# Peyton-Chen/RegionE

Hardware: AMD Instinct MI355X
Metric: denoising steps/sec (28-step RegionE edit, 1024x1024) (higher is better)
Workload: dtype bf16

## Files before the change

### regione_amd/_lib.py

```python
from __future__ import annotations

import ctypes as C
import os

import torch

from . import build as _build
from .build import LIB_PATH

LIB_PATH = os.environ.get("RGN_LIB", LIB_PATH)

_c_void_p, _c_int, _c_float = C.c_void_p, C.c_int, C.c_float



class QkvEpilogue(C.Structure):
    _fields_ = [("wq", _c_void_p), ("wk", _c_void_p), ("cos_q", _c_void_p), ("sin_q", _c_void_p), ("cos_k", _c_void_p),
                ("sin_k", _c_void_p), ("kv_rows", _c_void_p), ("k_slab", _c_void_p), ("vt_slab", _c_void_p),
                ("row_base", _c_int), ("skv_pad", _c_int), ("k_col", _c_int), ("v_col", _c_int), ("q_col", _c_int),
                ("heads", _c_int), ("eps", _c_float), ("fp16_roundtrip", _c_int)]


_qkv_p = C.POINTER(QkvEpilogue)

# ... 135 lines not shown
    "rgn_mmdit_double_block": [_block_p, _c_void_p],
    "rgn_mmdit_single_block": [_block_p, _c_void_p],
    "rgn_mmdit_block_bytes": [],
    "rgn_lora_merge_bf16": [_c_void_p, _c_int, _c_void_p, _c_int, _c_int, _c_int, _term_p, _c_int, _c_void_p],
    "rgn_image_resample_u8": [_c_void_p, _c_int, _c_int, _c_void_p, _c_int, _c_int, _c_void_p, _c_void_p, _c_int, _c_int, _c_void_p],
    "rgn_image_u8_to_nchw_bf16": [_c_void_p, _c_void_p, _c_int, _c_int, _c_void_p, _c_void_p],
    "rgn_image_patchify_u8": [_c_void_p, _c_int, _c_int, _c_void_p, _c_void_p, _c_int, _c_int, _c_void_p],
    "rgn_image_bf16_to_u8": [_c_void_p, _c_int, _c_int, _c_void_p, _c_int, _c_int, _c_void_p],
}
_RESTYPE = {"rgn_last_error": C.c_char_p, "rgn_abi_struct_bytes": C.c_size_t, "rgn_attention_workspace_bytes": C.c_size_t,
            "rgn_gemm_workspace_bytes": C.c_size_t, "rgn_groupnorm_workspace_bytes": C.c_size_t,
            "rgn_groupnorm_partial_bytes": C.c_size_t, "rgn_lm_decode_attention_workspace_bytes": C.c_size_t,
            "rgn_lm_head_workspace_bytes": C.c_size_t, "rgn_lm_pick_workspace_bytes": C.c_size_t,
            "rgn_rowband_side_launches": C.c_longlong, "rgn_mmdit_block_bytes": C.c_size_t}

_lib = None


class RegionEHipError(RuntimeError):
    pass


def lib():
    global _lib
    if _lib is not None:
        return _lib
    if not os.path.exists(LIB_PATH):
        raise RegionEHipError(
            f"{LIB_PATH} not found: the HIP extension is not built. Run "
            "`python -c 'import __graft_entry__ as g; g.build()'` (needs hipcc); there is no CPU fallback.")
    if os.path.abspath(LIB_PATH) == os.path.abspath(_build.LIB_PATH) and os.path.isdir(_build.CSRC):
        built, now = _build.built_from(), _build.csrc_hash()
        if built and built != now:
            raise RegionEHipError(f"{LIB_PATH} was built from kernel sources {built}, the tree holds {now}: rebuild with "
                                  "`python -m regione_amd.build` (or `__graft_entry__.build()`)")
    h = C.CDLL(LIB_PATH)
    for name, argtypes in SIGNATURES.items():
        fn = getattr(h, name)
        fn.argtypes = argtypes
        fn.restype = _RESTYPE.get(name, C.c_int)
    want = C.sizeof(QkvEpilogue) * 1000 + C.sizeof(GemmProblem)
    if h.rgn_abi_struct_bytes() != want:
        raise RegionEHipError(f"{LIB_PATH}: struct layout {h.rgn_abi_struct_bytes()} != the Python binding's {want} "
                              f"(library ABI version {h.rgn_version()}): rebuild with `python -m regione_amd.build --force`")
    if h.rgn_mmdit_block_bytes() != C.sizeof(MmditBlock):
        raise RegionEHipError(f"{LIB_PATH}: sizeof(rgn_mmdit_block) {h.rgn_mmdit_block_bytes()} != the Python binding's {C.sizeof(MmditBlock)}: "
                              "rebuild with `python -m regione_amd.build --force`")
    _lib = h
    return h


import contextlib as _contextlib

PLAN_KEYS = ("gemm_pieces", "gemm_geometry", "gemm_asm", "gemm_quarter", "attn_waves", "attn_split", "attn_streamk", "attn_asm", "rowbands")


@_contextlib.contextmanager
def plan_override(**knobs):
    h = lib()
    before = {}
    try:
        for k, v in knobs.items():
            old = C.c_int(-1)
            check(h.rgn_plan_override_get(k.encode(), C.byref(old)), f"rgn_plan_override_get({k})")
            check(h.rgn_plan_override(k.encode(), int(v)), f"rgn_plan_override({k})")
            before[k] = old.value
        yield
    finally:
        for k, old in before.items():
            h.rgn_plan_override(k.encode(), old)


def check(rc: int, what: str = ""):
    if rc != 0:
        msg = lib().rgn_last_error().decode(errors="replace")
        raise RegionEHipError(f"{what or 'libregione_hip'} failed (rc={rc}): {msg}")
```

### regione_amd/csrc/attn.hip

```cpp
#include "common.h"
#include <stdlib.h>
#include <utility>
#include "attn_loop_asm.inc"

namespace rgn {

typedef __attribute__((ext_vector_type(8))) __bf16 bf8_t;
typedef __attribute__((ext_vector_type(2))) __bf16 bf2_t;
typedef __attribute__((ext_vector_type(2))) float f32x2;
typedef __attribute__((address_space(3))) void* lds_ptr_t;
typedef const __attribute__((address_space(1))) void* glb_ptr_t;

struct AttnArgs {
    const uint16_t* Q;
    const uint16_t* K;
    const uint16_t* Vt;
    uint16_t* O;
    int ldq, ldo, skv_pad, Sq, Skv, H;
    float scale_log2e;
    int item_offset, nitems_launch, nsplit;
    int static_on;
    float static_m;
    float* ws;
};
// ... 368 lines not shown
                         : RGN_ATTN_LOOP_CLOBBERS);
        }
    }
    const float l_other = __shfl_xor(l_run, 32, 64);
    const float l_tot = l_run + l_other;
    if (SPLIT) {
        const size_t slot = SPLIT == 2 ? (size_t)unit * 2 + seg : (size_t)(item - g.item_offset) * g.nsplit + split;
        float* base = g.ws + slot * (size_t)(QB * 130);
        float* orow = base + (size_t)(wave * 32 + ql) * 128;
        static_for<16>([&](auto Ic) {
            constexpr int I = decltype(Ic)::value;
            constexpr int db = I / 4, r4 = I % 4;
            *(float4*)(orow + db * 32 + 8 * r4 + 4 * half) =
                make_float4(agpr_read1<db * 16 + r4 * 4 + 0>(), agpr_read1<db * 16 + r4 * 4 + 1>(),
                            agpr_read1<db * 16 + r4 * 4 + 2>(), agpr_read1<db * 16 + r4 * 4 + 3>());
        });
        if (half == 0) {
            base[QB * 128 + wave * 32 + ql] = m_run;
            base[QB * 129 + wave * 32 + ql] = l_tot;
        }
        if (SPLIT != 2) return;
        sk_lo += ntiles;
        ++seg;
        if (sk_lo >= sk_hi) return;
        __syncthreads();
        continue;
    }
    const float inv = 1.0f / l_tot;
    constexpr int OT_LD = 136;
    uint16_t* ot = (uint16_t*)smem;
    {
        uint16_t* orow = ot + (wave * 32 + ql) * OT_LD;
        static_for<16>([&](auto Ic) {
            constexpr int I = decltype(Ic)::value;
            constexpr int db = I / 4, r4 = I % 4;
            const int d = db * 32 + 8 * r4 + 4 * half;
            const uint32_t w0 = cvt_pk_bf16(agpr_read1<db * 16 + r4 * 4 + 0>() * inv, agpr_read1<db * 16 + r4 * 4 + 1>() * inv);
            const uint32_t w1 = cvt_pk_bf16(agpr_read1<db * 16 + r4 * 4 + 2>() * inv, agpr_read1<db * 16 + r4 * 4 + 3>() * inv);
            *(uint2*)(orow + d) = make_uint2(w0, w1);
        });
    }
    __syncthreads();
    constexpr int RPP = 512 / 16;
#pragma unroll
    for (int it = 0; it < QB / RPP; ++it) {
        const int row = (tid >> 4) + it * RPP, c = (tid & 15) * 8;
        const int qr2 = qb * QB + row;
        if (qr2 < g.Sq) *(uint4*)(g.O + (size_t)qr2 * g.ldo + h * 128 + c) = *(const uint4*)(ot + row * OT_LD + c);
    }
    return;
  }
}

__global__ __launch_bounds__(256, 1) void attention_asm64_kernel(const AttnArgs g) {
    constexpr int QB = 256;
    extern __shared__ __attribute__((aligned(16))) uint8_t smem[];
    const int tid = threadIdx.x;
    const int wave = __builtin_amdgcn_readfirstlane(tid >> 6);
    const int nQ = (g.Sq + QB - 1) / QB;
    const int ntiles = g.Skv / KV_T;
    int unit;
    {
        const int nb = g.nitems_launch;
        const int bid = blockIdx.x, xcd = bid & 7, loc = bid >> 3;
        const int q = nb >> 3, r = nb & 7;
        unit = (xcd < r ? xcd * (q + 1) : r * (q + 1) + (xcd - r) * q) + loc;
    }
    const uint32_t HD2 = (uint32_t)g.H * 256u;
    const int lane = tid & 63;
    const int ql = lane & 31, half = lane >> 5;
    const int item = g.item_offset + unit;
    const int h = item / nQ, qb = item - h * nQ;
    const int q0 = qb * QB + wave * 64;
    float m_run = g.static_m, l_run0 = 0.f, l_run1 = 0.f;
    {
        uint32_t krel[8], vrel[4];
#pragma unroll
        for (int ks = 0; ks < 8; ++ks) krel[ks] = ql * 256 + (((ks * 2 + half) ^ (ql & 15)) << 4);
#pragma unroll
        for (int kb4 = 0; kb4 < 4; ++kb4) vrel[kb4] = ql * 128 + (((kb4 * 2 + half) ^ ((ql >> 1) & 7)) << 4);
        uint32_t dk[4], dv[4];
#pragma unroll
        for (int p = 0; p < 4; ++p) {
            const int piece = wave * 4 + p;
            const int krow = piece * 4 + (lane >> 4);
            dk[p] = (uint32_t)krow * HD2 + h * 256 + (((lane & 15) ^ (krow & 15)) << 4);
            const int vrow = piece * 8 + (lane >> 3);
            dv[p] = (uint32_t)(h * 128 + vrow) * (uint32_t)(g.skv_pad * 2) + (((lane & 7) ^ ((vrow >> 1) & 7)) << 4);
        }
        const uint16_t* qptr0 = g.Q + (size_t)min(q0 + ql, g.Sq - 1) * g.ldq + h * 128 + half * 8;
        const uint16_t* qptr1 = g.Q + (size_t)min(q0 + 32 + ql, g.Sq - 1) * g.ldq + h * 128 + half * 8;
        auto rsrc = [](const void* p) {
            const uint64_t a = (uint64_t)p;
            u32x4_s r;
            r[0] = __builtin_amdgcn_readfirstlane((uint32_t)a);
            r[1] = __builtin_amdgcn_readfirstlane((uint32_t)(a >> 32) & 0xffffu);
            r[2] = 0xffffffffu;
            r[3] = 0x00020000u;
            return r;
        };
        const u32x4_s rk = rsrc(g.K), rv = rsrc(g.Vt);
        const uint32_t lds0 = (uint32_t)(uintptr_t)(__attribute__((address_space(3))) uint8_t*)smem;
        const uint32_t kadv = __builtin_amdgcn_readfirstlane((uint32_t)KV_T * HD2);
        uint32_t tk = __builtin_amdgcn_readfirstlane(0u), tv = __builtin_amdgcn_readfirstlane(0u);
        const uint32_t tk_last = __builtin_amdgcn_readfirstlane((uint32_t)(ntiles - 1) * kadv);
        const uint32_t tv_last = __builtin_amdgcn_readfirstlane((uint32_t)(ntiles - 1) * 128u);
        uint32_t stg_k = __builtin_amdgcn_readfirstlane(lds0 + 32768u), stg_v = __builtin_amdgcn_readfirstlane(lds0), stg_d = stg_v;
        const uint32_t wdst = __builtin_amdgcn_readfirstlane((uint32_t)wave * 4096u);
        uint32_t cnt = __builtin_amdgcn_readfirstlane((uint32_t)(ntiles - 1) >> 1), rem = __builtin_amdgcn_readfirstlane((uint32_t)(ntiles - 1) & 1u);
        const float sl2e = g.scale_log2e;
        uint32_t stmp, stmp2, sdst;
        asm volatile(RGN_ATTN_LOOP_W64_ASM
                     : [l_run0] "+&v"(l_run0), [l_run1] "+&v"(l_run1), [tk] "+&s"(tk), [tv] "+&s"(tv), [stg_k] "+&s"(stg_k),
                       [stg_v] "+&s"(stg_v), [stg_d] "+&s"(stg_d), [cnt] "+&s"(cnt), [stmp] "=&s"(stmp), [stmp2] "=&s"(stmp2),
                       [sdst] "=&s"(sdst)
                     : [krel0] "v"(krel[0]), [krel1] "v"(krel[1]), [krel2] "v"(krel[2]), [krel3] "v"(krel[3]), [krel4] "v"(krel[4]),
                       [krel5] "v"(krel[5]), [krel6] "v"(krel[6]), [krel7] "v"(krel[7]), [vrel0] "v"(vrel[0]), [vrel1] "v"(vrel[1]),
                       [vrel2] "v"(vrel[2]), [vrel3] "v"(vrel[3]), [dk0] "v"(dk[0]), [dk1] "v"(dk[1]), [dk2] "v"(dk[2]), [dk3] "v"(dk[3]),
                       [dv0] "v"(dv[0]), [dv1] "v"(dv[1]), [dv2] "v"(dv[2]), [dv3] "v"(dv[3]), [qptr0] "v"(qptr0), [qptr1] "v"(qptr1),
                       [m_run] "v"(m_run), [rk] "s"(rk), [rv] "s"(rv), [kadv] "s"(kadv), [tk_last] "s"(tk_last), [tv_last] "s"(tv_last),
                       [wdst] "s"(wdst), [rem] "s"(rem), [sl2e] "s"(sl2e)
                     : RGN_ATTN_LOOP_W64_CLOBBERS);
    }
    const float inv0 = 1.0f / (l_run0 + __shfl_xor(l_run0, 32, 64));
    const float inv1 = 1.0f / (l_run1 + __shfl_xor(l_run1, 32, 64));
    constexpr int OT_LD = 136;
    uint16_t* ot = (uint16_t*)smem;
    static_for<32>([&](auto Ic) {
        constexpr int I = decltype(Ic)::value;
        constexpr int j = I / 16, db = (I / 4) % 4, r4 = I % 4, A = j * 64 + db * 16 + r4 * 4;
        const float inv = j ? inv1 : inv0;
        uint16_t* orow = ot + ((wave * 2 + j) * 32 + ql) * OT_LD;
        const int d = db * 32 + 8 * r4 + 4 * half;
        const uint32_t w0 = cvt_pk_bf16(agpr_read1<A + 0>() * inv, agpr_read1<A + 1>() * inv);
        const uint32_t w1 = cvt_pk_bf16(agpr_read1<A + 2>() * inv, agpr_read1<A + 3>() * inv);
        *(uint2*)(orow + d) = make_uint2(w0, w1);
    });
    __syncthreads();
    constexpr int RPP = 256 / 16;
#pragma unroll
    for (int it = 0; it < QB / RPP; ++it) {
        const int row = (tid >> 4) + it * RPP, c = (tid & 15) * 8;
        const int qr2 = qb * QB + row;
        if (qr2 < g.Sq) *(uint4*)(g.O + (size_t)qr2 * g.ldo + h * 128 + c) = *(const uint4*)(ot + row * OT_LD + c);
    }
}

template <int QB>
__global__ __launch_bounds__(256) void attention_combine_kernel(const AttnArgs g) {
    const int nQ = (g.Sq + QB - 1) / QB;
    const int u = blockIdx.x / (QB / 16);
    const int row = (blockIdx.x % (QB / 16)) * 16 + (threadIdx.x >> 4);
    const int c = (threadIdx.x & 15) * 8;
    const int item = g.item_offset + u;
    const int h = item / nQ, qb = item - h * nQ;
    const int qr = qb * QB + row;
    if (qr >= g.Sq) return;
    const float* base = g.ws + (size_t)u * g.nsplit * (size_t)(QB * 130);
    float mstar = -1e30f;
    for (int s = 0; s < g.nsplit; ++s) mstar = fmaxf(mstar, base[(size_t)s * QB * 130 + QB * 128 + row]);
    float acc[8] = {0.f, 0.f, 0.f, 0.f, 0.f, 0.f, 0.f, 0.f};
    float l = 0.f;
    for (int s = 0; s < g.nsplit; ++s) {
        const float* b = base + (size_t)s * QB * 130;
        const float w = __builtin_amdgcn_exp2f(b[QB * 128 + row] - mstar);
        l += b[QB * 129 + row] * w;
        const float4 x0 = *(const float4*)(b + (size_t)row * 128 + c), x1 = *(const float4*)(b + (size_t)row * 128 + c + 4);
        acc[0] += x0.x * w; acc[1] += x0.y * w; acc[2] += x0.z * w; acc[3] += x0.w * w;
        acc[4] += x1.x * w; acc[5] += x1.y * w; acc[6] += x1.z * w; acc[7] += x1.w * w;
    }
    const float inv = 1.0f / l;
    uint4 out;
    out.x = cvt_pk_bf16(acc[0] * inv, acc[1] * inv); out.y = cvt_pk_bf16(acc[2] * inv, acc[3] * inv);
    out.z = cvt_pk_bf16(acc[4] * inv, acc[5] * inv); out.w = cvt_pk_bf16(acc[6] * inv, acc[7] * inv);
    *(uint4*)(g.O + (size_t)qr * g.ldo + h * 128 + c) = out;
}

template <int QB>
__global__ __launch_bounds__(256) void attention_combine_sk_kernel(const AttnArgs g, int G) {
    const int nQ = (g.Sq + QB - 1) / QB;
    const int u = blockIdx.x / (QB / 16);
    const int row = (blockIdx.x % (QB / 16)) * 16 + (threadIdx.x >> 4);
    const int c = (threadIdx.x & 15) * 8;
    const int item = g.item_offset + u;
    const int h = item / nQ, qb = item - h * nQ;
    const int qr = qb * QB + row;
    if (qr >= g.Sq) return;
    const int nt = g.Skv / KV_T;
    const long long total = (long long)g.nitems_launch * nt;
    const long long lo = (long long)u * nt, hi = lo + nt;
    auto bound = [&](int w) { return (long long)w * total / G; };
    int w0 = (int)(lo * G / total);
    while (w0 + 1 < G && bound(w0 + 1) <= lo) ++w0;
    while (w0 > 0 && bound(w0) > lo) --w0;
    float mstar = -1e30f;
    for (int w = w0; w < G && bound(w) < hi; ++w) {
        if (bound(w + 1) <= bound(w)) continue;
        const int sg = ((int)(bound(w) / nt) == u) ? 0 : 1;
        mstar = fmaxf(mstar, g.ws[((size_t)w * 2 + sg) * (size_t)(QB * 130) + QB * 128 + row]);
    }
    float acc[8] = {0.f, 0.f, 0.f, 0.f, 0.f, 0.f, 0.f, 0.f};
    float l = 0.f;
    for (int w = w0; w < G && bound(w) < hi; ++w) {
        if (bound(w + 1) <= bound(w)) continue;
        const int sg = ((int)(bound(w) / nt) == u) ? 0 : 1;
        const float* b = g.ws + ((size_t)w * 2 + sg) * (size_t)(QB * 130);
        const float wt = __builtin_amdgcn_exp2f(b[QB * 128 + row] - mstar);
        l += b[QB * 129 + row] * wt;
        const float4 x0 = *(const float4*)(b + (size_t)row * 128 + c), x1 = *(const float4*)(b + (size_t)row * 128 + c + 4);
        acc[0] += x0.x * wt; acc[1] += x0.y * wt; acc[2] += x0.z * wt; acc[3] += x0.w * wt;
        acc[4] += x1.x * wt; acc[5] += x1.y * wt; acc[6] += x1.z * wt; acc[7] += x1.w * wt;
    }
    const float inv = 1.0f / l;
    uint4 out;
    out.x = cvt_pk_bf16(acc[0] * inv, acc[1] * inv); out.y = cvt_pk_bf16(acc[2] * inv, acc[3] * inv);
    out.z = cvt_pk_bf16(acc[4] * inv, acc[5] * inv); out.w = cvt_pk_bf16(acc[6] * inv, acc[7] * inv);
    *(uint4*)(g.O + (size_t)qr * g.ldo + h * 128 + c) = out;
}

template <int SPLIT>
static int launch_attention_asm(const AttnArgs& g, int nblocks, hipStream_t st) {
    constexpr int LDS = 5 * ATT_STAGE;
    static bool attr[64] = {};
    int dev = 0;
    (void)hipGetDevice(&dev);
    if (dev < 0 || dev >= 64 || !attr[dev]) {
        (void)hipFuncSetAttribute((const void*)attention_asm_kernel<SPLIT, false>, hipFuncAttributeMaxDynamicSharedMemorySize, LDS);
        (void)hipFuncSetAttribute((const void*)attention_asm_kernel<SPLIT, true>, hipFuncAttributeMaxDynamicSharedMemorySize, LDS);
        if (SPLIT == 0) (void)hipFuncSetAttribute((const void*)attention_asm64_kernel, hipFuncAttributeMaxDynamicSharedMemorySize, LDS);
        if (dev >= 0 && dev < 64) attr[dev] = true;
    }
    if (nblocks == 0) return 0;
    if (SPLIT == 0 && g.static_on) hipLaunchKernelGGL(attention_asm64_kernel, dim3(nblocks), dim3(256), LDS, st, g);
    else if (g.static_on) hipLaunchKernelGGL((attention_asm_kernel<SPLIT, true>), dim3(nblocks), dim3(512), LDS, st, g);
    else hipLaunchKernelGGL((attention_asm_kernel<SPLIT, false>), dim3(nblocks), dim3(512), LDS, st, g);
    return check_launch("attention_asm_kernel");
}

static bool attention_use_asm(const AttnArgs& g) {
    return plan_override().attn_asm != 0 && (g.Skv % KV_T) == 0 && (size_t)g.skv_pad * g.H * 256 < ((size_t)1 << 32);
}

template <int NW, int NSTAGE, bool SPLIT>
static int launch_attention(const AttnArgs& g, hipStream_t st) {
    if (NW == 8 && attention_use_asm(g))
        return launch_attention_asm<SPLIT ? 1 : 0>(g, SPLIT ? g.nitems_launch * g.nsplit : g.nitems_launch, st);
    constexpr int LDS = NSTAGE * ATT_STAGE;
    static bool attr[64] = {};
    int dev = 0;
    (void)hipGetDevice(&dev);
    if (dev < 0 || dev >= 64 || !attr[dev]) {
        (void)hipFuncSetAttribute((const void*)attention_kernel<NW, NSTAGE, SPLIT>, hipFuncAttributeMaxDynamicSharedMemorySize, LDS);
        if (dev >= 0 && dev < 64) attr[dev] = true;
    }
    const int nblocks = SPLIT ? g.nitems_launch * g.nsplit : g.nitems_launch;
    if (nblocks == 0) return 0;
    hipLaunchKernelGGL((attention_kernel<NW, NSTAGE, SPLIT>), dim3(nblocks), dim3(64 * NW), LDS, st, g);
    return check_launch("attention_kernel");
}

static thread_local int g_last_attn_plan = 0;

template <int NW, int NSTAGE>
static int attention_schedule(AttnArgs g, int slots, void* ws, size_t ws_bytes, hipStream_t st, bool dry = false) {
    constexpr int QB = 32 * NW;
    const int nitems = g.H * ((g.Sq + QB - 1) / QB);
    const int ntiles = (g.Skv + KV_T - 1) / KV_T;
    int full = (nitems / slots) * slots, left = nitems - full, best = 1;
    const float c_t = NW == 8 ? 1.69f : 0.95f, c_p = 10.7f, c_m = 8.0f;
    float best_cost = (float)((left + slots - 1) / slots) * ((float)ntiles * c_t + c_p);
    if (NW == 8 && full == 0 && left > 0) {
        const float x = fmaxf(0.0f, (float)(left - 72) / 184.0f);
        best_cost = (float)ntiles * (1.10f + 0.59f * x * x) + c_p;
    }
    bool stream_k = false;
    if (left > 0 && ws != nullptr) {
        for (int S = 2; S <= 8; ++S) {
            if (ntiles / S < 4) break;
            if ((size_t)left * S * QB * 130 * sizeof(float) > ws_bytes) break;
            const float cost = (float)((left * S + slots - 1) / slots) * ((float)((ntiles + S - 1) / S) * c_t + c_p) + c_m;
            if (cost < best_cost - 1e-3f) { best_cost = cost; best = S; }
        }
        const int sk_o = plan_override().attn_streamk;
        const long long steps = (long long)left * ntiles;
        if (NW == 8 && sk_o != 0 && attention_use_asm(g) && left < slots && steps >= 8LL * slots &&
            (size_t)slots * 2 * QB * 130 * sizeof(float) <= ws_bytes) {
            const float cost = (float)((steps + slots - 1) / slots) * c_t + 2.0f * c_p + c_m;
            if (cost < best_cost - 1e-3f || sk_o == 1) { best_cost = cost; stream_k = true; }
        }
    }
    g_last_attn_plan = (stream_k ? 1 : best) | (stream_k ? 0x10 : 0) | (NW == 8 ? 0x20 : 0);
    if (dry) return 0;
    g.ws = (float*)ws;
    g.nsplit = 1;
    int rc = 0;
    if (stream_k) {
        if (full > 0) {
            g.item_offset = 0; g.nitems_launch = full;
            if ((rc = launch_attention<NW, NSTAGE, false>(g, st))) return rc;
        }
        g.item_offset = full; g.nitems_launch = left;
        if ((rc = launch_attention_asm<2>(g, slots, st))) return rc;
        hipLaunchKernelGGL((attention_combine_sk_kernel<QB>), dim3(left * (QB / 16)), dim3(256), 0, st, g, slots);
        return check_launch("attention_combine_sk_kernel");
    }
    if (best == 1) {
        g.item_offset = 0; g.nitems_launch = nitems;
        return launch_attention<NW, NSTAGE, false>(g, st);
    }
    if (full > 0) {
        g.item_offset = 0; g.nitems_launch = full;
        if ((rc = launch_attention<NW, NSTAGE, false>(g, st))) return rc;
    }
    g.item_offset = full; g.nitems_launch = left; g.nsplit = best;
    if ((rc = launch_attention<NW, NSTAGE, true>(g, st))) return rc;
    hipLaunchKernelGGL((attention_combine_kernel<QB>), dim3(left * (QB / 16)), dim3(256), 0, st, g);
    return check_launch("attention_combine_kernel");
}

}

using namespace rgn;

extern "C" {

size_t rgn_attention_workspace_bytes(int Sq, int H) {
    (void)Sq; (void)H;
    return (size_t)128 << 20;
}

int rgn_attention(const void* Q, int ldq, const void* k_slab, const void* vt_slab, int skv_pad, void* O, int ldo,
                  int Sq, int Skv, int H, float scale, void* workspace, size_t workspace_bytes, void* stream) {
    return rgn_attention_bounded(Q, ldq, k_slab, vt_slab, skv_pad, O, ldo, Sq, Skv, H, scale, 0.0f, workspace, workspace_bytes, stream);
}

int rgn_attention_bounded(const void* Q, int ldq, const void* k_slab, const void* vt_slab, int skv_pad, void* O, int ldo,
                          int Sq, int Skv, int H, float scale, float score_bound, void* workspace, size_t workspace_bytes,
                          void* stream) {
    if (Sq == 0) return 0;
    if (!Q || !k_slab || !vt_slab || !O || Sq < 0 || Skv <= 0 || H <= 0 || (skv_pad % 64) || skv_pad < Skv ||
        (ldq % 8) || (ldo % 8))
        return fail(RGN_E_BADARG, "attention: bad argument");
    AttnArgs g;
    g.Q = (const uint16_t*)Q; g.K = (const uint16_t*)k_slab; g.Vt = (const uint16_t*)vt_slab; g.O = (uint16_t*)O;
    g.ldq = ldq; g.ldo = ldo; g.skv_pad = skv_pad; g.Sq = Sq; g.Skv = Skv; g.H = H;
    g.scale_log2e = scale * 1.4426950408889634f;
    g.item_offset = 0; g.nitems_launch = 0; g.nsplit = 1; g.ws = nullptr;
    {
        const float b2 = score_bound * 1.4426950408889634f;
        g.static_on = (score_bound > 0.0f && b2 <= 96.0f) ? 1 : 0;
        g.static_m = 0.0f;
    }
    hipStream_t st = (hipStream_t)stream;
    int variant = (H * ((Sq + 255) / 256) >= 96) ? 8 : 4;
    const PlanOverride& ov = plan_override();
    if (ov.attn_waves == 4 || ov.attn_waves == 8) variant = ov.attn_waves;
    if (ov.attn_split == 0) { workspace = nullptr; workspace_bytes = 0; }
    if (variant == 8) return attention_schedule<8, 3>(g, 256, workspace, workspace_bytes, st);
    return attention_schedule<4, 2>(g, 512, workspace, workspace_bytes, st);
}

int rgn_attention_last_plan(void) { return g_last_attn_plan; }

int rgn_attention_plan_query(int Sq, int Skv, int H, size_t workspace_bytes) {
    if (Sq <= 0 || Skv <= 0 || H <= 0) return fail(RGN_E_BADARG, "attention_plan_query: bad argument");
    AttnArgs g{};
    g.Sq = Sq; g.Skv = Skv; g.H = H; g.skv_pad = (Skv + 63) / 64 * 64;
    int variant = (H * ((Sq + 255) / 256) >= 96) ? 8 : 4;
// ... 10 lines not shown
```

### regione_amd/csrc/common.h

```cpp
#pragma once
#include <hip/hip_runtime.h>
#include <stdint.h>
#include <stdio.h>

#include "../../include/regione_hip.h"

namespace rgn {

extern thread_local char g_err[256];

inline int fail(int code, const char* msg) {
    snprintf(g_err, sizeof(g_err), "%s", msg);
    return code;
}

inline int check_launch(const char* what) {
    hipError_t e = hipGetLastError();
    if (e != hipSuccess) {
        snprintf(g_err, sizeof(g_err), "%s: %s", what, hipGetErrorString(e));
        return (int)e;
    }
    return 0;
}

typedef __attribute__((ext_vector_type(2))) __bf16 hw_bf16x2;
typedef __attribute__((ext_vector_type(2))) float hw_f32x2;
__device__ __forceinline__ uint32_t f2bf_pk(float lo, float hi) {
    hw_bf16x2 r = __builtin_convertvector(hw_f32x2{lo, hi}, hw_bf16x2);
    return __builtin_bit_cast(uint32_t, r);
}
__device__ __forceinline__ uint16_t f2bf(float f) { return (uint16_t)f2bf_pk(f, 0.f); }
__device__ __forceinline__ float bf2f(uint16_t h) { return __uint_as_float(((uint32_t)h) << 16); }
__device__ __forceinline__ float rbf(float f) { return __uint_as_float(f2bf_pk(f, 0.f) << 16); }

__device__ __forceinline__ float wave_sum(float v) {
#pragma unroll
    for (int o = 32; o > 0; o >>= 1) v += __shfl_xor(v, o, 64);
    return v;
}

struct PlanOverride {
    int gemm_pieces;
    int gemm_geometry;
    int gemm_asm;
    int gemm_quarter;
    int attn_waves;
    int attn_split;
    int attn_streamk;
    int attn_asm;
    int rowbands;
};
PlanOverride& plan_override();

bool rowband_active(hipStream_t st, hipStream_t* side);
void rowband_count_side_launch();
bool rowband_cut(const int* Ms, const uintptr_t* addr, int n, int* which, int* row);

typedef __attribute__((ext_vector_type(8))) short bf16x8;
typedef __attribute__((ext_vector_type(4))) float f32x4;
typedef __attribute__((ext_vector_type(16))) float f32x16;

}
```

### regione_amd/csrc/region.hip

```cpp
#include "common.h"
#include <stdlib.h>
#include <string.h>

namespace rgn {

thread_local char g_err[256] = "";

template <typename T> __device__ __forceinline__ float ld_as_f32(const T* p, size_t i);
template <> __device__ __forceinline__ float ld_as_f32<float>(const float* p, size_t i) { return p[i]; }
template <> __device__ __forceinline__ float ld_as_f32<uint16_t>(const uint16_t* p, size_t i) { return bf2f(p[i]); }

__device__ __forceinline__ float row_sum_torch(float p, int lane) {
    const int j = lane & 7;
    const float t = p + __shfl_xor(p, 32, 64);
    const float a = ((__shfl(t, j, 64) + __shfl(t, 8 + j, 64)) + __shfl(t, 16 + j, 64)) + __shfl(t, 24 + j, 64);
    float s = __shfl(a, 0, 64);
#pragma unroll
    for (int l = 1; l < 8; ++l) s = s + __shfl(a, l, 64);
    return s;
}

__device__ __forceinline__ float row_sumsq_torch_f32(float x, int lane) {
    const int j = lane & 7;
    const float x0 = __shfl(x, j, 64);
// ... 196 lines not shown
        float f = nrm;
        if (nrm > 1.0f) f = rnd<T>((float)pow((double)nrm, (double)rnd<T>(power)));
        else if (nrm < 1.0f) f = 1.0f;
        sd = rnd<T>(sd / f);
    }
    float c = rnd<T>(__fadd_rn(n, sd));
    if (mode == 2) {
        const float cn = row_norm(p);
        const float nn = row_norm(c);
        c = rnd<T>(__fmul_rn(c, rnd<T>(cn / nn)));
    }
    st_from_f32<T>(out, i, c);
}

static inline int grid_for(size_t n, int block) {
    size_t g = (n + block - 1) / block;
    return (int)(g < 1 ? 1 : (g > 2048 ? 2048 : g));
}

template <typename TS, typename TM>
static int launch_sim(const void* sample, const void* mo, const void* cond, int cond_dtype, float dt_final,
                      float thr, int L, uint8_t* raw, float* sim, hipStream_t st) {
    dim3 g((L + 3) / 4), b(256);
    if (cond_dtype == RGN_BF16)
        hipLaunchKernelGGL((arp_sim_kernel<TS, TM, uint16_t>), g, b, 0, st, (const TS*)sample, (const TM*)mo,
                           (const uint16_t*)cond, dt_final, thr, L, raw, sim);
    else
        hipLaunchKernelGGL((arp_sim_kernel<TS, TM, float>), g, b, 0, st, (const TS*)sample, (const TM*)mo,
                           (const float*)cond, dt_final, thr, L, raw, sim);
    return check_launch("arp_sim_kernel");
}

static int launch_morph(const uint8_t* raw, int H, int W, int ed, int64_t* e, int64_t* u, uint8_t* mask,
                        int32_t* count, hipStream_t st) {
    const int L = H * W;
    const size_t lds = 2 * (size_t)((L + 15) & ~15);
    if (lds > 150 * 1024) return fail(RGN_E_UNSUPPORTED, "arp: token grid larger than 76800 tokens");
    if (lds > 64 * 1024)
        (void)hipFuncSetAttribute((const void*)arp_morph_compact_kernel, hipFuncAttributeMaxDynamicSharedMemorySize, 150 * 1024);
    hipLaunchKernelGGL(arp_morph_compact_kernel, dim3(1), dim3(1024), lds, st, raw, H, W, ed, e, u, mask, count);
    return check_launch("arp_morph_compact_kernel");
}

__global__ void sel_rows_kernel(const int64_t* __restrict__ ids, int K, int T, int64_t* __restrict__ out) {
    const int i = blockIdx.x * blockDim.x + threadIdx.x;
    if (i < T) out[i] = i;
    else if (i < T + K) out[i] = (int64_t)T + ids[i - T];
}

static int* plan_field(PlanOverride& o, const char* key) {
    struct { const char* name; int* field; } tab[] = {
        {"gemm_pieces", &o.gemm_pieces}, {"gemm_geometry", &o.gemm_geometry}, {"gemm_asm", &o.gemm_asm}, {"gemm_quarter", &o.gemm_quarter},
        {"attn_waves", &o.attn_waves}, {"attn_split", &o.attn_split}, {"attn_streamk", &o.attn_streamk}, {"attn_asm", &o.attn_asm},
        {"rowbands", &o.rowbands}};
    for (auto& t : tab)
        if (strcmp(t.name, key) == 0) return t.field;
    return nullptr;
}

static bool plan_set(PlanOverride& o, const char* key, int value) {
    int* f = plan_field(o, key);
    if (f != nullptr) *f = value;
    return f != nullptr;
}

PlanOverride& plan_override() {
    static PlanOverride o = [] {
        PlanOverride v{-1, -1, -1, -1, -1, -1, -1, -1, -1};
        const char* e = getenv("RGN_PLAN_OVERRIDE");
        if (e != nullptr) {
            char buf[256];
            snprintf(buf, sizeof(buf), "%s", e);
            char* save = nullptr;
            for (char* tok = strtok_r(buf, ",", &save); tok != nullptr; tok = strtok_r(nullptr, ",", &save)) {
                char* eq = strchr(tok, '=');
                if (eq != nullptr) *eq = 0;
                if (eq == nullptr || !plan_set(v, tok, atoi(eq + 1))) fprintf(stderr, "regione_hip: RGN_PLAN_OVERRIDE: bad entry '%s'\n", tok);
            }
        }
        return v;
    }();
    return o;
}

struct RowBandState {
    hipStream_t side = nullptr, main = nullptr;
    hipEvent_t forked = nullptr, joined = nullptr;
    bool on = false;
};
static thread_local RowBandState g_rowband[64];
static thread_local long long g_rowband_side_launches = 0;

static RowBandState* rowband_state() {
    int dev = 0;
    if (hipGetDevice(&dev) != hipSuccess || dev < 0 || dev >= 64) return nullptr;
    return &g_rowband[dev];
}

bool rowband_active(hipStream_t st, hipStream_t* side) {
    RowBandState* s = rowband_state();
    if (s == nullptr || !s->on || s->main != st) return false;
    *side = s->side;
    return true;
}

void rowband_count_side_launch() { ++g_rowband_side_launches; }

bool rowband_cut(const int* Ms, const uintptr_t* addr, int n, int* which, int* row) {
    int total = 0, best = -1;
    for (int i = 0; i < n; ++i) {
        if (Ms[i] <= 0) continue;
        total += (Ms[i] + 255) / 256;
        if (best < 0 || Ms[i] > Ms[best] || (Ms[i] == Ms[best] && (addr == nullptr || addr[i] >= addr[best]))) best = i;
    }
    if (best < 0) return false;
    const int mine = (Ms[best] + 255) / 256, others = total - mine;
    if (mine < 2) return false;
    const int pct = plan_override().rowbands;
    const int share = (pct >= 2 && pct <= 98) ? pct : 50;
    int k = (total * share + 50) / 100 - others;
    k = k < 1 ? 1 : (k > mine - 1 ? mine - 1 : k);
// ... 20 lines not shown
        e = hipStreamCreateWithFlags(&side, hipStreamNonBlocking);
        if (e == hipSuccess) e = hipEventCreateWithFlags(&a, hipEventDisableTiming);
        if (e == hipSuccess) e = hipEventCreateWithFlags(&b, hipEventDisableTiming);
        if (e != hipSuccess) return fail((int)e, hipGetErrorString(e));
        s->side = side; s->forked = a; s->joined = b;
    }
    e = hipEventRecord(s->forked, (hipStream_t)stream);
    if (e == hipSuccess) e = hipStreamWaitEvent(s->side, s->forked, 0);
    if (e != hipSuccess) return fail((int)e, hipGetErrorString(e));
    s->main = (hipStream_t)stream;
    s->on = true;
    return 0;
}

int rgn_rowband_join(void* stream) {
    RowBandState* s = rowband_state();
    if (s == nullptr || !s->on) return 0;
    if (s->main != (hipStream_t)stream) return fail(RGN_E_BADARG, "rowband_join: another stream was forked");
    s->on = false;
    hipError_t e = hipEventRecord(s->joined, s->side);
    if (e == hipSuccess) e = hipStreamWaitEvent((hipStream_t)stream, s->joined, 0);
    return e == hipSuccess ? 0 : fail((int)e, hipGetErrorString(e));
}

int rgn_rowband_query(const int* Ms, int nprob, int* cut_problem, int* cut_row) {
    if (!Ms || nprob < 1 || nprob > 4 || !cut_problem || !cut_row) return fail(RGN_E_BADARG, "rowband_query: 1..4 problems");
    for (int i = 0; i < nprob; ++i)
        if (Ms[i] < 0) return fail(RGN_E_BADARG, "rowband_query: negative row count");
    *cut_problem = -1; *cut_row = 0;
    return rowband_cut(Ms, nullptr, nprob, cut_problem, cut_row) ? 1 : 0;
}

long long rgn_rowband_side_launches(void) { return g_rowband_side_launches; }

int rgn_version(void) { return RGN_ABI_VERSION; }
size_t rgn_abi_struct_bytes(void) { return sizeof(rgn_qkv_epilogue) * 1000 + sizeof(rgn_gemm_problem); }

int rgn_sel_rows(const int64_t* edited_ids, int K, int T, int64_t* out, void* stream) {
    if (K < 0 || T < 0 || (K > 0 && !edited_ids) || !out) return fail(RGN_E_BADARG, "sel_rows: bad argument");
    if (T + K == 0) return 0;
    hipLaunchKernelGGL(sel_rows_kernel, dim3((T + K + 255) / 256), dim3(256), 0, (hipStream_t)stream, edited_ids, K, T, out);
    return check_launch("sel_rows_kernel");
}

int rgn_fill_zero(void* ptr, size_t bytes, void* stream) {
    if (bytes == 0) return 0;
    if (!ptr) return fail(RGN_E_BADARG, "fill_zero: null pointer");
    hipError_t e = hipMemsetAsync(ptr, 0, bytes, (hipStream_t)stream);
    return e == hipSuccess ? 0 : fail((int)e, hipGetErrorString(e));
}

int rgn_plan_override(const char* key, int value) {
    PlanOverride& o = plan_override();
    if (key == nullptr) { o = PlanOverride{-1, -1, -1, -1, -1, -1, -1, -1, -1}; return 0; }
    return plan_set(o, key, value) ? 0 : fail(RGN_E_BADARG, "plan_override: unknown key");
}
int rgn_plan_override_get(const char* key, int* value) {
    int* f = key != nullptr ? plan_field(plan_override(), key) : nullptr;
    if (f == nullptr || value == nullptr) return fail(RGN_E_BADARG, "plan_override_get: unknown key");
    *value = *f;
    return 0;
}
const char* rgn_last_error(void) { return g_err; }

int rgn_device_info(int* cu_count, int* clock_khz, size_t* hbm_bytes) {
    hipDeviceProp_t p;
    int dev = 0;
    hipError_t e = hipGetDevice(&dev);
    if (e == hipSuccess) e = hipGetDeviceProperties(&p, dev);
    if (e != hipSuccess) return fail((int)e, hipGetErrorString(e));
    if (cu_count) *cu_count = p.multiProcessorCount;
    if (clock_khz) *clock_khz = p.clockRate;
    if (hbm_bytes) *hbm_bytes = p.totalGlobalMem;
    return 0;
}

int rgn_arp_partition(const void* sample, int sample_dtype, const void* model_output, int mo_dtype,
                      const void* cond, int cond_dtype, float dt_final, float threshold, int L, int D, int h_tok,
                      int w_tok, int erosion_dilation, int64_t* edited_ids, int64_t* unedited_ids,
                      uint8_t* raw_mask, uint8_t* mask, float* sim_out, int32_t* count, void* stream) {
    if (D != 64) return fail(RGN_E_UNSUPPORTED, "arp: latent width must be 64");
    if (L <= 0 || h_tok * w_tok != L) return fail(RGN_E_BADARG, "arp: h_tok*w_tok != L");
    if (!sample || !cond || !edited_ids || !unedited_ids || !raw_mask || !mask || !count)
        return fail(RGN_E_BADARG, "arp: null pointer");
    hipStream_t st = (hipStream_t)stream;
    int rc;
    const bool sb = sample_dtype == RGN_BF16, mb = mo_dtype == RGN_BF16;
    if (sb && mb) rc = launch_sim<uint16_t, uint16_t>(sample, model_output, cond, cond_dtype, dt_final, threshold, L, raw_mask, sim_out, st);
    else if (sb) rc = launch_sim<uint16_t, float>(sample, model_output, cond, cond_dtype, dt_final, threshold, L, raw_mask, sim_out, st);
    else if (mb) rc = launch_sim<float, uint16_t>(sample, model_output, cond, cond_dtype, dt_final, threshold, L, raw_mask, sim_out, st);
    else rc = launch_sim<float, float>(sample, model_output, cond, cond_dtype, dt_final, threshold, L, raw_mask, sim_out, st);
    if (rc) return rc;
    return launch_morph(raw_mask, h_tok, w_tok, erosion_dilation, edited_ids, unedited_ids, mask, count, st);
}

int rgn_morph_compact(const uint8_t* raw_mask, int h_tok, int w_tok, int erosion_dilation, int64_t* edited_ids,
                      int64_t* unedited_ids, uint8_t* mask, int32_t* count, void* stream) {
    if (!raw_mask || !edited_ids || !unedited_ids || !mask || !count || h_tok <= 0 || w_tok <= 0)
        return fail(RGN_E_BADARG, "morph_compact: bad argument");
    return launch_morph(raw_mask, h_tok, w_tok, erosion_dilation, edited_ids, unedited_ids, mask, count,
                        (hipStream_t)stream);
}

static int rows_op(const void* src, const int64_t* ids, void* dst, int K, int row_bytes, bool scatter, void* stream) {
    if (K == 0) return 0;
    if (!src || !ids || !dst || K < 0 || row_bytes <= 0 || (row_bytes & 3)) return fail(RGN_E_BADARG, "rows: bad argument");
    hipStream_t st = (hipStream_t)stream;
// ... 63 lines not shown
```

Before: 21.30.

## Run split-KV and stream-K attention through the wave64 asm kernel with static-max combine

Templates the 256-thread asm64 attention kernel on split mode, so split-KV and stream-K launches can use it. Stream-K units may loop over two segments and write partial outputs and row sums to a workspace. When a static softmax max is in use, the combine kernels skip the max reduction and exponential rescaling and simply sum the partials. The split chooser also skips split counts that would leave an empty tail split. This adds a new override knob, with risk around the static-max precision assumption and the correctness of the workspace layout.

```diff
diff --git a/regione_amd/_lib.py b/regione_amd/_lib.py
--- a/regione_amd/_lib.py
+++ b/regione_amd/_lib.py
@@ -211,7 +211,8 @@
 
 import contextlib as _contextlib
 
-PLAN_KEYS = ("gemm_pieces", "gemm_geometry", "gemm_asm", "gemm_quarter", "attn_waves", "attn_split", "attn_streamk", "attn_asm", "rowbands")
+PLAN_KEYS = ("gemm_pieces", "gemm_geometry", "gemm_asm", "gemm_quarter", "attn_waves", "attn_split", "attn_streamk", "attn_asm", "rowbands",
+             "attn_split_w64")
 
 
 @_contextlib.contextmanager
diff --git a/regione_amd/csrc/attn.hip b/regione_amd/csrc/attn.hip
--- a/regione_amd/csrc/attn.hip
+++ b/regione_amd/csrc/attn.hip
@@ -444,24 +444,50 @@
   }
 }
 
+template <int SPLIT>
 __global__ __launch_bounds__(256, 1) void attention_asm64_kernel(const AttnArgs g) {
     constexpr int QB = 256;
     extern __shared__ __attribute__((aligned(16))) uint8_t smem[];
     const int tid = threadIdx.x;
     const int wave = __builtin_amdgcn_readfirstlane(tid >> 6);
     const int nQ = (g.Sq + QB - 1) / QB;
-    const int ntiles = g.Skv / KV_T;
-    int unit;
+    const int ntiles_all = g.Skv / KV_T;
+    int unit, split = 0;
     {
-        const int nb = g.nitems_launch;
+        const int nb = SPLIT == 2 ? (int)gridDim.x : SPLIT == 1 ? g.nitems_launch * g.nsplit : g.nitems_launch;
         const int bid = blockIdx.x, xcd = bid & 7, loc = bid >> 3;
         const int q = nb >> 3, r = nb & 7;
         unit = (xcd < r ? xcd * (q + 1) : r * (q + 1) + (xcd - r) * q) + loc;
     }
+    int sk_lo = 0, sk_hi = 0, seg = 0;
+    if (SPLIT == 2) {
+        const long long total = (long long)g.nitems_launch * ntiles_all;
+        sk_lo = (int)((long long)unit * total / (int)gridDim.x);
+        sk_hi = (int)((long long)(unit + 1) * total / (int)gridDim.x);
+        if (sk_lo >= sk_hi) return;
+    }
     const uint32_t HD2 = (uint32_t)g.H * 256u;
-    const int lane = tid & 63;
+#pragma nounroll
+  for (;;) {
+    int lane = tid & 63;
+    if (SPLIT == 2) asm volatile("" : "+v"(lane));
     const int ql = lane & 31, half = lane >> 5;
-    const int item = g.item_offset + unit;
+    int item, t_begin = 0, ntiles = ntiles_all;
+    if (SPLIT == 2) {
+        const int il = sk_lo / ntiles_all;
+        item = g.item_offset + il;
+        t_begin = sk_lo - il * ntiles_all;
+        ntiles = min(ntiles_all - t_begin, sk_hi - sk_lo);
+    } else if (SPLIT == 1) {
+        split = unit % g.nsplit;
+        item = g.item_offset + unit / g.nsplit;
+        const int per = (ntiles_all + g.nsplit - 1) / g.nsplit;
+        t_begin = split * per;
+        ntiles = min(per, ntiles_all - t_begin);
+        if (ntiles <= 0) return;
+    } else {
+        item = g.item_offset + unit;
+    }
     const int h = item / nQ, qb = item - h * nQ;
     const int q0 = qb * QB + wave * 64;
     float m_run = g.static_m, l_run0 = 0.f, l_run1 = 0.f;
@@ -494,9 +520,9 @@
         const u32x4_s rk = rsrc(g.K), rv = rsrc(g.Vt);
         const uint32_t lds0 = (uint32_t)(uintptr_t)(__attribute__((address_space(3))) uint8_t*)smem;
         const uint32_t kadv = __builtin_amdgcn_readfirstlane((uint32_t)KV_T * HD2);
-        uint32_t tk = __builtin_amdgcn_readfirstlane(0u), tv = __builtin_amdgcn_readfirstlane(0u);
-        const uint32_t tk_last = __builtin_amdgcn_readfirstlane((uint32_t)(ntiles - 1) * kadv);
-        const uint32_t tv_last = __builtin_amdgcn_readfirstlane((uint32_t)(ntiles - 1) * 128u);
+        uint32_t tk = __builtin_amdgcn_readfirstlane((uint32_t)t_begin * kadv), tv = __builtin_amdgcn_readfirstlane((uint32_t)t_begin * 128u);
+        const uint32_t tk_last = __builtin_amdgcn_readfirstlane((uint32_t)(t_begin + ntiles - 1) * kadv);
+        const uint32_t tv_last = __builtin_amdgcn_readfirstlane((uint32_t)(t_begin + ntiles - 1) * 128u);
         uint32_t stg_k = __builtin_amdgcn_readfirstlane(lds0 + 32768u), stg_v = __builtin_amdgcn_readfirstlane(lds0), stg_d = stg_v;
         const uint32_t wdst = __builtin_amdgcn_readfirstlane((uint32_t)wave * 4096u);
         uint32_t cnt = __builtin_amdgcn_readfirstlane((uint32_t)(ntiles - 1) >> 1), rem = __builtin_amdgcn_readfirstlane((uint32_t)(ntiles - 1) & 1u);
@@ -514,8 +540,31 @@
                        [wdst] "s"(wdst), [rem] "s"(rem), [sl2e] "s"(sl2e)
                      : RGN_ATTN_LOOP_W64_CLOBBERS);
     }
-    const float inv0 = 1.0f / (l_run0 + __shfl_xor(l_run0, 32, 64));
-    const float inv1 = 1.0f / (l_run1 + __shfl_xor(l_run1, 32, 64));
+    const float l_tot0 = l_run0 + __shfl_xor(l_run0, 32, 64);
+    const float l_tot1 = l_run1 + __shfl_xor(l_run1, 32, 64);
+    if (SPLIT) {
+        const size_t slot = SPLIT == 2 ? (size_t)unit * 2 + seg : (size_t)(item - g.item_offset) * g.nsplit + split;
+        float* base = g.ws + slot * (size_t)(QB * 130);
+        static_for<32>([&](auto Ic) {
+            constexpr int I = decltype(Ic)::value;
+            constexpr int j = I / 16, db = (I / 4) % 4, r4 = I % 4, A = j * 64 + db * 16 + r4 * 4;
+            float* orow = base + (size_t)((wave * 2 + j) * 32 + ql) * 128;
+            *(float4*)(orow + db * 32 + 8 * r4 + 4 * half) =
+                make_float4(agpr_read1<A + 0>(), agpr_read1<A + 1>(), agpr_read1<A + 2>(), agpr_read1<A + 3>());
+        });
+        if (half == 0) {
+            base[QB * 129 + wave * 64 + ql] = l_tot0;
+            base[QB * 129 + wave * 64 + 32 + ql] = l_tot1;
+        }
+        if (SPLIT != 2) return;
+        sk_lo += ntiles;
+        ++seg;
+        if (sk_lo >= sk_hi) return;
+        __syncthreads();
+        continue;
+    }
+    const float inv0 = 1.0f / l_tot0;
+    const float inv1 = 1.0f / l_tot1;
     constexpr int OT_LD = 136;
     uint16_t* ot = (uint16_t*)smem;
     static_for<32>([&](auto Ic) {
@@ -536,6 +585,8 @@
         const int qr2 = qb * QB + row;
         if (qr2 < g.Sq) *(uint4*)(g.O + (size_t)qr2 * g.ldo + h * 128 + c) = *(const uint4*)(ot + row * OT_LD + c);
     }
+    return;
+  }
 }
 
 template <int QB>
@@ -550,9 +601,19 @@
     if (qr >= g.Sq) return;
     const float* base = g.ws + (size_t)u * g.nsplit * (size_t)(QB * 130);
     float mstar = -1e30f;
-    for (int s = 0; s < g.nsplit; ++s) mstar = fmaxf(mstar, base[(size_t)s * QB * 130 + QB * 128 + row]);
+    if (!g.static_on)
+        for (int s = 0; s < g.nsplit; ++s) mstar = fmaxf(mstar, base[(size_t)s * QB * 130 + QB * 128 + row]);
     float acc[8] = {0.f, 0.f, 0.f, 0.f, 0.f, 0.f, 0.f, 0.f};
     float l = 0.f;
+    if (g.static_on) {
+        for (int s = 0; s < g.nsplit; ++s) {
+            const float* b = base + (size_t)s * QB * 130;
+            l += b[QB * 129 + row];
+            const float4 x0 = *(const float4*)(b + (size_t)row * 128 + c), x1 = *(const float4*)(b + (size_t)row * 128 + c + 4);
+            acc[0] += x0.x; acc[1] += x0.y; acc[2] += x0.z; acc[3] += x0.w;
+            acc[4] += x1.x; acc[5] += x1.y; acc[6] += x1.z; acc[7] += x1.w;
+        }
+    } else
     for (int s = 0; s < g.nsplit; ++s) {
         const float* b = base + (size_t)s * QB * 130;
         const float w = __builtin_amdgcn_exp2f(b[QB * 128 + row] - mstar);
@@ -586,13 +647,24 @@
     while (w0 + 1 < G && bound(w0 + 1) <= lo) ++w0;
     while (w0 > 0 && bound(w0) > lo) --w0;
     float mstar = -1e30f;
-    for (int w = w0; w < G && bound(w) < hi; ++w) {
+    for (int w = w0; !g.static_on && w < G && bound(w) < hi; ++w) {
         if (bound(w + 1) <= bound(w)) continue;
         const int sg = ((int)(bound(w) / nt) == u) ? 0 : 1;
         mstar = fmaxf(mstar, g.ws[((size_t)w * 2 + sg) * (size_t)(QB * 130) + QB * 128 + row]);
     }
     float acc[8] = {0.f, 0.f, 0.f, 0.f, 0.f, 0.f, 0.f, 0.f};
     float l = 0.f;
+    if (g.static_on) {
+        for (int w = w0; w < G && bound(w) < hi; ++w) {
+            if (bound(w + 1) <= bound(w)) continue;
+            const int sg = ((int)(bound(w) / nt) == u) ? 0 : 1;
+            const float* b = g.ws + ((size_t)w * 2 + sg) * (size_t)(QB * 130);
+            l += b[QB * 129 + row];
+            const float4 x0 = *(const float4*)(b + (size_t)row * 128 + c), x1 = *(const float4*)(b + (size_t)row * 128 + c + 4);
+            acc[0] += x0.x; acc[1] += x0.y; acc[2] += x0.z; acc[3] += x0.w;
+            acc[4] += x1.x; acc[5] += x1.y; acc[6] += x1.z; acc[7] += x1.w;
+        }
+    } else
     for (int w = w0; w < G && bound(w) < hi; ++w) {
         if (bound(w + 1) <= bound(w)) continue;
         const int sg = ((int)(bound(w) / nt) == u) ? 0 : 1;
@@ -610,6 +682,8 @@
     *(uint4*)(g.O + (size_t)qr * g.ldo + h * 128 + c) = out;
 }
 
+static bool attention_split_w64() { return plan_override().attn_split_w64 != 0; }
+
 template <int SPLIT>
 static int launch_attention_asm(const AttnArgs& g, int nblocks, hipStream_t st) {
     constexpr int LDS = 5 * ATT_STAGE;
@@ -619,11 +693,11 @@
     if (dev < 0 || dev >= 64 || !attr[dev]) {
         (void)hipFuncSetAttribute((const void*)attention_asm_kernel<SPLIT, false>, hipFuncAttributeMaxDynamicSharedMemorySize, LDS);
         (void)hipFuncSetAttribute((const void*)attention_asm_kernel<SPLIT, true>, hipFuncAttributeMaxDynamicSharedMemorySize, LDS);
-        if (SPLIT == 0) (void)hipFuncSetAttribute((const void*)attention_asm64_kernel, hipFuncAttributeMaxDynamicSharedMemorySize, LDS);
+        (void)hipFuncSetAttribute((const void*)attention_asm64_kernel<SPLIT>, hipFuncAttributeMaxDynamicSharedMemorySize, LDS);
         if (dev >= 0 && dev < 64) attr[dev] = true;
     }
     if (nblocks == 0) return 0;
-    if (SPLIT == 0 && g.static_on) hipLaunchKernelGGL(attention_asm64_kernel, dim3(nblocks), dim3(256), LDS, st, g);
+    if (g.static_on && (SPLIT == 0 || attention_split_w64())) hipLaunchKernelGGL(attention_asm64_kernel<SPLIT>, dim3(nblocks), dim3(256), LDS, st, g);
     else if (g.static_on) hipLaunchKernelGGL((attention_asm_kernel<SPLIT, true>), dim3(nblocks), dim3(512), LDS, st, g);
     else hipLaunchKernelGGL((attention_asm_kernel<SPLIT, false>), dim3(nblocks), dim3(512), LDS, st, g);
     return check_launch("attention_asm_kernel");
@@ -669,6 +743,7 @@
     if (left > 0 && ws != nullptr) {
         for (int S = 2; S <= 8; ++S) {
             if (ntiles / S < 4) break;
+            if ((S - 1) * ((ntiles + S - 1) / S) >= ntiles) continue;
             if ((size_t)left * S * QB * 130 * sizeof(float) > ws_bytes) break;
             const float cost = (float)((left * S + slots - 1) / slots) * ((float)((ntiles + S - 1) / S) * c_t + c_p) + c_m;
             if (cost < best_cost - 1e-3f) { best_cost = cost; best = S; }
@@ -693,6 +768,7 @@
         }
         g.item_offset = full; g.nitems_launch = left;
         if ((rc = launch_attention_asm<2>(g, slots, st))) return rc;
+        if (!attention_split_w64()) g.static_on = 0;
         hipLaunchKernelGGL((attention_combine_sk_kernel<QB>), dim3(left * (QB / 16)), dim3(256), 0, st, g, slots);
         return check_launch("attention_combine_sk_kernel");
     }
@@ -706,6 +782,7 @@
     }
     g.item_offset = full; g.nitems_launch = left; g.nsplit = best;
     if ((rc = launch_attention<NW, NSTAGE, true>(g, st))) return rc;
+    if (!(NW == 8 && attention_use_asm(g) && attention_split_w64())) g.static_on = 0;
     hipLaunchKernelGGL((attention_combine_kernel<QB>), dim3(left * (QB / 16)), dim3(256), 0, st, g);
     return check_launch("attention_combine_kernel");
 }
diff --git a/regione_amd/csrc/common.h b/regione_amd/csrc/common.h
--- a/regione_amd/csrc/common.h
+++ b/regione_amd/csrc/common.h
@@ -49,6 +49,7 @@
     int attn_streamk;
     int attn_asm;
     int rowbands;
+    int attn_split_w64;
 };
 PlanOverride& plan_override();
 
diff --git a/regione_amd/csrc/region.hip b/regione_amd/csrc/region.hip
--- a/regione_amd/csrc/region.hip
+++ b/regione_amd/csrc/region.hip
@@ -272,7 +272,7 @@
     struct { const char* name; int* field; } tab[] = {
         {"gemm_pieces", &o.gemm_pieces}, {"gemm_geometry", &o.gemm_geometry}, {"gemm_asm", &o.gemm_asm}, {"gemm_quarter", &o.gemm_quarter},
         {"attn_waves", &o.attn_waves}, {"attn_split", &o.attn_split}, {"attn_streamk", &o.attn_streamk}, {"attn_asm", &o.attn_asm},
-        {"rowbands", &o.rowbands}};
+        {"rowbands", &o.rowbands}, {"attn_split_w64", &o.attn_split_w64}};
     for (auto& t : tab)
         if (strcmp(t.name, key) == 0) return t.field;
     return nullptr;
@@ -286,7 +286,7 @@
 
 PlanOverride& plan_override() {
     static PlanOverride o = [] {
-        PlanOverride v{-1, -1, -1, -1, -1, -1, -1, -1, -1};
+        PlanOverride v{-1, -1, -1, -1, -1, -1, -1, -1, -1, -1};
         const char* e = getenv("RGN_PLAN_OVERRIDE");
         if (e != nullptr) {
             char buf[256];
@@ -413,7 +413,7 @@
 
 int rgn_plan_override(const char* key, int value) {
     PlanOverride& o = plan_override();
-    if (key == nullptr) { o = PlanOverride{-1, -1, -1, -1, -1, -1, -1, -1, -1}; return 0; }
+    if (key == nullptr) { o = PlanOverride{-1, -1, -1, -1, -1, -1, -1, -1, -1, -1}; return 0; }
     return plan_set(o, key, value) ? 0 : fail(RGN_E_BADARG, "plan_override: unknown key");
 }
 int rgn_plan_override_get(const char* key, int* value) {
```

Result: no change. 21.39, median of 6 (+0.4%).
